# danieleschmidt/Photonic-Flash-Attention

Measured on AMD Instinct MI355X. Metric: attention_fwd_tflops, higher is better.
Workload: dtype bf16; 1 GPU; C3: B=4/GPU S=4096 H=16 D=128 bf16 causal (BASELINE.json configs[2], the headline shape); global_batch=4, seq_len=4096, heads=16, head_dim=128, causal=True, kernel=fa3_fwd_p4_bf16_d128_causal_o16, workgroups=256

## Files before the change

### include/pfa_hip.h

```cpp
#ifndef PFA_HIP_H
#define PFA_HIP_H

#include <stddef.h>
#include <stdint.h>

#ifdef __cplusplus
extern "C" {
#endif

#define PFA_ABI_VERSION 9

typedef enum pfa_status {
    PFA_OK = 0,
    PFA_ERR_NULL = -1,
    PFA_ERR_STRUCT_SIZE = -2,
    PFA_ERR_SHAPE = -3,
    PFA_ERR_HEAD_DIM = -4,
    PFA_ERR_DTYPE = -5,
    PFA_ERR_STRIDE = -6,
    PFA_ERR_ALIGN = -7,
    PFA_ERR_DEVICE = -8,
    PFA_ERR_LAUNCH = -9,
    PFA_ERR_FLAGS = -10
} pfa_status;

typedef enum pfa_dtype {
    PFA_DTYPE_BF16 = 0,
    PFA_DTYPE_FP16 = 1,
    PFA_DTYPE_FP32 = 2
} pfa_dtype;

#define PFA_FLAG_SPLIT_P   0x1u
#define PFA_FLAG_NO_XCD_MAP 0x2u
#define PFA_FLAG_VARIANT_MASK 0xff00u

typedef struct pfa_fa3_args {
    uint32_t size;
    uint32_t flags;

    const void* q;
    const void* k;
    const void* v;
    void*       o;
    float*      lse;
    const int32_t* seqlens_k;
    const uint8_t* key_mask;

    int64_t q_stride_b, q_stride_h, q_stride_s;
    int64_t k_stride_b, k_stride_h, k_stride_s;
    int64_t v_stride_b, v_stride_h, v_stride_s;
    int64_t o_stride_b, o_stride_h, o_stride_s;
    int64_t key_mask_stride_b;

    int32_t B, H, Sq, Sk, D;
    int32_t dtype_in;
    int32_t dtype_out;
// ... 304 lines not shown
```

### photonic_flash_attention_amd/_capi.py

```python

from __future__ import annotations

import ctypes as C
import os
import threading
from typing import Optional

PFA_ABI_VERSION = 9
PFA_DTYPE_BF16, PFA_DTYPE_FP16, PFA_DTYPE_FP32 = 0, 1, 2
PFA_FLAG_SPLIT_P = 0x1
PFA_FLAG_NO_XCD_MAP = 0x2
PFA_ROPE_INTERLEAVED = 0x1
PFA_MERGE_MAX_PARTS = 8
PFA_PREFILL_MAX_SPLITS = 8

_PKG_DIR = os.path.dirname(os.path.abspath(__file__))
LIB_PATH = os.path.join(_PKG_DIR, "libpfa_hip.so")

class PfaFa3Args(C.Structure):
    _fields_ = [
        ("size", C.c_uint32), ("flags", C.c_uint32),
        ("q", C.c_void_p), ("k", C.c_void_p), ("v", C.c_void_p), ("o", C.c_void_p),
        ("lse", C.c_void_p), ("seqlens_k", C.c_void_p), ("key_mask", C.c_void_p),
        ("q_stride_b", C.c_int64), ("q_stride_h", C.c_int64), ("q_stride_s", C.c_int64),
        ("k_stride_b", C.c_int64), ("k_stride_h", C.c_int64), ("k_stride_s", C.c_int64),
        ("v_stride_b", C.c_int64), ("v_stride_h", C.c_int64), ("v_stride_s", C.c_int64),
        ("o_stride_b", C.c_int64), ("o_stride_h", C.c_int64), ("o_stride_s", C.c_int64),
        ("key_mask_stride_b", C.c_int64),
        ("B", C.c_int32), ("H", C.c_int32), ("Sq", C.c_int32), ("Sk", C.c_int32), ("D", C.c_int32),
        ("dtype_in", C.c_int32), ("dtype_out", C.c_int32), ("causal", C.c_int32),
        ("softmax_scale", C.c_float), ("device_id", C.c_int32),
        ("workspace", C.c_void_p), ("workspace_bytes", C.c_size_t),
        ("mask", C.c_void_p),
        ("mask_stride_b", C.c_int64), ("mask_stride_h", C.c_int64), ("mask_stride_q", C.c_int64),
# ... 332 lines not shown
```

### photonic_flash_attention_amd/csrc/gen_fa3_fwd_p4.py

```python
#!/usr/bin/env python3
import os
import sys


DEV = os.environ.get("P4_DEV", "") == "1"
_stray = sorted(k for k in os.environ if k.startswith("P4_") and not (DEV and k in ("P4_DEV", "P4_STAMP")))
if _stray:
    sys.exit(f"gen_fa3_fwd_p4.py: {', '.join(_stray)} set without P4_DEV=1 -- the product code object takes no experiment knobs" if not DEV else
             f"gen_fa3_fwd_p4.py: unknown knob {', '.join(_stray)} -- P4_STAMP is the only one (with P4_DEV=1)")


def knob(name, default):
    return os.environ.get(name, default) if DEV else default


KA = dict(q=0, k=2, v=4, o=6, lse=8, q_sb=10, q_sh=11, k_sb=12, k_sh=13, v_sb=14, v_sh=15, o_sb=16, o_sh=17,
          q_ss=18, k_ss=19, v_ss=20, o_ss=21, H=22, Sq=23, Sk=24, NB=25, NU=26, magic_NU=27, magic_H=28, kv_group=29,
          magic_G=30, scale_log2=31, thr=32, hx=33, xcd_mode=34, SL=35, nt_full=36, pad=37, dbg=38)
KARG_DWORDS = 40
KARG_MEM_DWORDS = 42
KA_SEQLENS = 40
KBASE_SGPR = 60


# ... 115 lines not shown
    def need(self, tags):
        idx = [self.q.index(t) for t in tags if t in self.q]
        if not idx:
            return None
        i = max(idx)
        n = len(self.q) - 1 - i
        self.q = self.q[i + 1:]
        return f"s_waitcnt lgkmcnt({n})"


class Gen:
    def __init__(self, dtype, causal, out32=False, split=False, D=128, kmask=False, klen=False):
        assert out32 == split, "the code object carries the fast variant (16-bit store, one P) and the parity variant (fp32 store, split P)"
        self.dt, self.causal, self.out32, self.split, self.kmask = dtype, causal, out32, split, kmask
        self.klen = klen
        assert not (kmask and klen)
        self.kleft, self.kleft0 = (S('L_n'), ka('Sk')) if causal else (S('n_sub'), S('L_n'))
        self.mwords = kmask or klen
        self.nd_n, self.nd = S('nd_n'), S('nd')
        self.Lcut = S('L_n') if klen else ka('nt_full')
        if kmask and causal:
            self.kleft0 = ka('nt_full')
        self.cl = (klen or kmask) and causal
        self.fast = not split
        self.ret = S('grow')
        assert not (kmask and STAMP), "the key-mask kernels keep their mask words where the stamps keep their clock (s[58:59], the dbg kernarg)"
        assert D in (64, 128)
        self.D, self.KS, self.DB = D, D // 16, D // 32
        self.NKF, self.NVF = 2 * self.KS, 4 * self.DB
        self.TILE = 128 * D
        self.HALF = self.TILE // 2
        self.K_BASE, self.V_BASE, self.Q_BASE, self.O_BASE = 0, 2 * self.TILE, 4 * self.TILE, 8 * self.TILE
        self.LDS_BYTES = 10 * self.TILE
        self.PPW = self.TILE // 4096
        self.RB, self.CPR = 2 * D, D // 8
        assert RING <= min(self.NKF, self.NVF)
        self.mf = "v_mfma_f32_32x32x16_bf16" if dtype == "bf16" else "v_mfma_f32_32x32x16_f16"
        self.cvt = "v_cvt_pk_bf16_f32" if dtype == "bf16" else "v_cvt_pk_f16_f32"
        self.name = f"fa3_fwd_p4_{dtype}_d{D}_{'causal' if causal else 'full'}{'_km' if kmask else ('_kl' if klen else '')}_{'splitp_o32' if out32 else 'o16'}"
        self.main, self.ool, self.ool2, self.lstack = [], [], [], []
        self.L = self.main
        self.uid = 0

    def OA(self, X, db, e=0):
        return (0 if X == 'A' else 16 * self.DB) + 16 * db + e

# ... 460 lines not shown
                        self.i(x)
                        lg.issue(('kn', x))
                    pending = pending[2:]
                if rec is not None:
                    rec.append(sum(self.price(x.strip()) for x in self.L[mark:] if not x.strip().startswith("v_mfma")))
                else:
                    self.emit(fillers[hs] if hs < len(fillers) else [])
                hs += 1
        for x in pending:
            self.i(x)
        return lg

    def run_phase(self, fn, stream, lg, **kw):
        import copy
        save, uid = self.L, self.uid
        self.L, rec = [], []
        fn(fillers=None, lg=copy.deepcopy(lg), rec=rec, **kw)
        self.L, self.uid = save, uid
        fillers, tail = self.pack(stream, rec, ngaps=len(rec))
        lg = fn(fillers=fillers, lg=lg, **kw)
        self.emit(tail)
        return lg

    def stream_top(self, p):
        l1, l2 = self.ul("kok"), self.ul("vok")
        self.i(f"s_cmp_lg_u32 {S('krem')}, 0")
        self.i(f"s_cbranch_scc1 {l1}")
        self.i(f"s_mov_b64 {S('ksrd', 0, 2)}, {S('ksrd_n')}")
        self.i(f"s_mov_b32 {S('koff')}, 0")
        self.i(f"s_mov_b32 {S('krem')}, {S('nt_n')}")
        if self.kmask:
            self.i(f"s_mul_i32 {ka('pad')}, {S('n_b')}, {ka('Sk')}")
            self.i(f"s_mov_b32 {self.kleft}, {self.kleft0}")
        if self.klen:
            self.i(f"s_mov_b32 {ka('pad')}, {S('L_n')}")
        self.lab(l1)
        if self.kmask:
            self.len_word(0, dst=S('t2'), left=self.kleft)
            self.i(f"s_mov_b64 exec, {S('t2')}")
            self.emit(self.mask_load())
            self.i("s_mov_b64 exec, -1")
        if self.klen:
            self.len_word(p)
        self.i(f"s_cmp_lg_u32 {S('vrem')}, 0")
        self.i(f"s_cbranch_scc1 {l2}")
        self.i(f"s_mov_b64 {S('vsrd', 0, 2)}, {S('vsrd_n')}")
        self.i(f"s_mov_b32 {S('voff')}, 0")
        self.i(f"s_mov_b32 {S('vrem')}, {S('nt_n')}")
        self.lab(l2)

    def capture(self, fn):
        save, self.L = self.L, []
        fn()
        out, self.L = self.L, save
        return [x[1:] if x.startswith("\t") else x for x in out]

    def stream_bottom(self, p, barrier=True):
        lq, lb = self.ul("q"), self.ul("bar")
        self.i(f"s_add_u32 {S('koff')}, {S('koff')}, {S('ktile')}")
        self.i(f"s_add_u32 {S('voff')}, {S('voff')}, {S('vtile')}")
        self.i(f"s_sub_u32 {S('krem')}, {S('krem')}, 1")
        self.i(f"s_sub_u32 {S('vrem')}, {S('vrem')}, 1")
        self.i(f"s_sub_u32 {S('wrem')}, {S('wrem')}, 1")
        if self.kmask:
            self.i(f"s_add_u32 {ka('pad')}, {ka('pad')}, 64")
        if self.klen:
            self.i(f"s_sub_u32 {ka('pad')}, {ka('pad')}, 64")
        self.i(f"s_cmp_lg_u32 {S('qrem')}, 0")
        self.i(f"s_cbranch_scc1 {lq}")
        self.i("s_waitcnt vmcnt(0)")
        self.lab(lb)
        if self.kmask:
            self.i(self.mask_word(p))
            self.km_len_and(p)
        if barrier:
            self.i("s_barrier")
        self.out_of_line(True)
        self.lab(lq)
        self.q_group()
        self.q_group()
        self.i("s_waitcnt vmcnt(8)")
        self.i(f"s_branch {lb}")
        self.out_of_line(False)
# ... 81 lines not shown
            self.i(f"s_cmp_eq_u32 {S('wrem')}, {self.nd if self.cl else 1}")
            self.i(f"s_cbranch_scc1 {lm}")
            self.lab(lr)
            self.out_of_line(True)
            self.lab(lm)
            self.mask_diag(1 - p)
            self.i(f"s_branch {lr}")
            self.out_of_line(False)
        if not self.fast:
            sta = self.interleave(self.start_stream('A', 1 - p), self.start_stream('B', 1 - p, alt=True))
            self.run_phase(self.phase_pv, sta, lg, p=p, dma_at={}, preissued=True)
            lr, lb = self.ul("rescale"), self.ul("rescaled")
            self.i(f"s_cmp_lg_u64 {S('grow')}, 0")
            self.i(f"s_cbranch_scc1 {lr}")
            self.lab(lb)
            self.out_of_line(True)
            self.lab(lr)
            self.rescale()
            self.i(f"s_branch {lb}")
            self.out_of_line(False)
            return
        sta = self.interleave(self.start_fast('A', 1 - p), self.start_fast('B', 1 - p))
        if lean:
            inline = [f"s_add_u32 {S('koff')}, {S('koff')}, {S('ktile')}", f"s_add_u32 {S('voff')}, {S('voff')}, {S('vtile')}"] + \
                     ([f"s_add_u32 {ka('pad')}, {ka('pad')}, 64"] if self.kmask else []) + ["s_waitcnt vmcnt(0)"] + \
                     ([self.mask_word(p)] if self.kmask else [])
        else:
            inline = self.capture(lambda: self.stream_bottom(p, barrier=False))
        mid = dict(gap=MID_BARRIER_GAP[self.D], inline=inline, kreads=self.kprefetch(p))
        self.run_phase(self.phase_pv, sta, lg, p=p, dma_at={}, preissued=True, mid=mid)

    def body_last(self, p):
        self.cm(f"LAST body, parity {p}: this wave's last tile -- finish(j), PV(j); nothing to prefetch for the wave itself")
        d = self.dma_plan(p, [2 * t for t in range(self.PPW)], [2 * self.PPW + 2 * t for t in range(self.PPW)])
        if self.fast:
            self.emit(self.finish_fast(p))
            self.fix_check(p)
            self.emit(self.lupd('A') + self.lupd('B'))
            self.i("s_nop 1")
            self.phase_pv(p, [[] for _ in range(2 * self.NVF)], d, strips="AB")
            return
        self.emit(self.finish_stream('A', p))
        self.i("s_nop 1")
        self.run_phase(self.phase_pv, self.finish_stream('B', p), Lgkm(), p=p, dma_at=d, strips="A")
        self.i("s_nop 1")
        self.phase_pv(p, [[] for _ in range(2 * self.NVF)], {}, strips="B")

# ... 566 lines not shown
            self.i(f"v_lshlrev_b32 {e2}, 4, {e2}")
            for d, ss in ((KDOFF(t), 'k_ss'), (VDOFF(t), 'v_ss')):
                self.i(f"v_mul_lo_u32 {e4}, {e3}, {ka(ss)}")
                self.i(f"v_add_u32 {e4}, {e4}, {e2}")
                self.i(f"v_subrev_u32 {vr(d)}, {1024 * t}, {e4}")
        self.i(f"s_lshl_b32 {S('t1')}, {W}, 6")
        for t in range(4):
            self.i(f"v_lshl_or_b32 {e2}, {e0}, 2, {t}")
            self.i(f"v_xor_b32 {e2}, {e2}, {e1}")
            self.i(f"v_add_u32 {e3}, {4 * t}, {e0}")
            self.i(f"v_lshrrev_b32 {e4}, 3, {e2}")
            self.i(f"v_lshl_add_u32 {e3}, {e3}, 1, {e4}")
            self.i(f"v_add_u32 {e3}, {S('t1')}, {e3}")
            self.i(f"v_and_b32 {e2}, 7, {e2}")
            self.i(f"v_lshlrev_b32 {e2}, 4, {e2}")
            self.i(f"v_mul_lo_u32 {e4}, {e3}, {ka('q_ss')}")
            self.i(f"v_add_u32 {e4}, {e4}, {e2}")
            self.i(f"v_subrev_u32 {vr(QDOFF(t))}, {1024 * t}, {e4}")

    def item_switch(self):
        self.i(f"s_mov_b32 {S('irem')}, {S('n_nt')}")
        self.i(f"s_sub_u32 {S('krem')}, {S('n_nt')}, 2")
        self.i(f"s_sub_u32 {S('vrem')}, {S('n_nt')}, 1")
        if self.cl:
            self.i(f"s_cmp_eq_u32 {self.nd_n}, 0")
            self.i(f"s_cselect_b32 {S('wrem')}, {S('wave')}, 3")
            self.i(f"s_cselect_b32 {self.nd}, 1, 0x80000000")
            self.i(f"s_add_u32 {S('wrem')}, {S('wrem')}, {S('n_nt')}")
            self.i(f"s_sub_u32 {S('wrem')}, {S('wrem')}, 4")
        elif self.causal:
            self.i(f"s_add_u32 {S('wrem')}, {S('n_nt')}, {S('wave')}")
            self.i(f"s_sub_u32 {S('wrem')}, {S('wrem')}, 4")
        else:
            self.i(f"s_sub_u32 {S('wrem')}, {S('n_nt')}, 1")
        self.make_out_srds()
        if self.causal:
            lone, ldone = self.ul("loneblock"), self.ul("advanced")
            self.i(f"s_lshl_b32 {S('t0')}, {S('n_qblk')}, 1")
            self.i(f"s_add_u32 {S('t0')}, {S('t0')}, 1")
            self.i(f"s_sub_u32 {S('t0')}, {S('t0')}, {ka('NB')}")
            self.i(f"s_or_b32 {S('t0')}, {S('t0')}, {S('n_sub')}")
            self.i(f"s_cmp_eq_u32 {S('t0')}, 0")
            self.i(f"s_cbranch_scc1 {lone}")
            self.i(f"s_xor_b32 {S('n_sub')}, {S('n_sub')}, 1")
            self.i(f"s_cmp_eq_u32 {S('n_sub')}, 0")
            self.i(f"s_cselect_b32 {S('t0')}, 1, 0")
            self.i(f"s_add_u32 {S('n_u')}, {S('n_u')}, {S('t0')}")
            self.i(f"s_branch {ldone}")
            self.lab(lone)
            self.i(f"s_add_u32 {S('n_u')}, {S('n_u')}, 1")
            self.lab(ldone)
        else:
            self.i(f"s_add_u32 {S('n_u')}, {S('n_u')}, 1")
        self.decode()
        self.i(f"s_mov_b32 {S('nt_n')}, {S('n_nt')}")
        self.i(f"s_lshl_b32 {S('qrem')}, {S('n_valid')}, {2 if self.PPW == 4 else 1}")
        self.i(f"s_lshl_b32 {S('qdst')}, {S('w4k')}, 2")
        self.i(f"s_add_u32 {S('qdst')}, {S('qdst')}, {self.Q_BASE}")
        self.i(f"s_mov_b32 {S('qoff')}, 0")

    def kernel(self):
        n = self.name
        self.L += [f"\t.globl\t{n}", "\t.p2align\t8", f"\t.type\t{n},@function", f"{n}:"]
        self.i(f"s_load_dwordx16 s[{KBASE_SGPR}:{KBASE_SGPR + 15}], s[0:1], 0")
        self.i(f"s_load_dwordx16 s[{KBASE_SGPR + 16}:{KBASE_SGPR + 31}], s[0:1], 64")
        self.i(f"s_load_dwordx8 s[{KBASE_SGPR + 32}:{KBASE_SGPR + 39}], s[0:1], 128")
        L, T0, T1, T2, T3 = vr(V_LANE), *(vr(x) for x in V_T)
        W = S('wave')
        self.i(f"v_and_b32 {L}, 63, v0")
        self.i(f"v_lshrrev_b32 {T0}, 6, v0")
        self.i("s_nop 0")
        self.i(f"v_readfirstlane_b32 {W}, {T0}")
        self.i("s_waitcnt lgkmcnt(0)")
        self.stamp_init()
        self.i(f"s_lshl_b32 {S('ktile')}, {ka('k_ss')}, 6")
        self.i(f"s_lshl_b32 {S('vtile')}, {ka('v_ss')}, 6")
        self.i(f"s_lshl_b32 {S('w4k')}, {W}, {12 if self.D == 128 else 11}")
        for sr, ss, rows in (('ksrd', 'k_ss', 'Sk'), ('vsrd', 'v_ss', 'Sk'), ('qsrd_n', 'q_ss', None), ('osrd', 'o_ss', None)):
# ... 26 lines not shown
        self.i(f"s_cbranch_scc1 {lend}")
        self.i(f"s_lshl_b32 {S('qdst')}, {S('w4k')}, 2")
        self.i(f"s_add_u32 {S('qdst')}, {S('qdst')}, {self.Q_BASE}")
        self.i(f"s_mov_b32 {S('qoff')}, 0")
        if self.kmask:
            self.i(f"s_mul_i32 {ka('pad')}, {S('n_b')}, {ka('Sk')}")
            self.emit(self.mask_load(0))
            self.i(f"s_add_u32 {ka('pad')}, {ka('pad')}, 64")
            self.emit(self.mask_load(1))
            self.i(f"s_add_u32 {ka('pad')}, {ka('pad')}, 64")
        if self.klen:
            self.i(f"s_mov_b32 {ka('pad')}, {S('L_n')}")
            self.len_word(0)
            self.i(f"s_sub_u32 {ka('pad')}, {ka('pad')}, 64")
            self.len_word(1)
            self.i(f"s_sub_u32 {ka('pad')}, {ka('pad')}, 64")
        self.i(f"s_mov_b32 {S('qrem')}, {self.PPW}")
        for g in range(self.PPW):
            self.q_group()
        self.i(f"s_mov_b64 {S('ksrd', 0, 2)}, {S('ksrd_n')}")
        self.i(f"s_mov_b64 {S('vsrd', 0, 2)}, {S('vsrd_n')}")
        self.i(f"s_mov_b32 {S('koff')}, 0")
        self.i(f"s_mov_b32 {S('voff')}, 0")
        self.i(self.setm0('k', 0))
        self.i("s_nop 0")
        for t in range(self.PPW):
            self.i(self.dma('K', t))
        self.i(self.setm0('v', 0))
        self.i("s_nop 0")
        for t in range(self.PPW):
            self.i(self.dma('V', t))
        self.i(f"s_add_u32 {S('koff')}, {S('koff')}, {S('ktile')}")
        self.i(self.setm0('k', 1))
        self.i("s_nop 0")
        for t in range(self.PPW):
            self.i(self.dma('K', t))
        self.i(f"s_add_u32 {S('koff')}, {S('koff')}, {S('ktile')}")
        self.i(f"s_add_u32 {S('voff')}, {S('voff')}, {S('vtile')}")
        self.i(f"s_waitcnt vmcnt({2 * self.PPW})")
        if self.kmask:
            self.i(self.mask_word(0, 0))
            self.i(self.mask_word(1, 1))
            self.i(f"s_mov_b32 {self.kleft}, {self.kleft0}")
            self.km_len_and(0)
            self.km_len_and(1)
        self.i("s_barrier")
        litem = f".L{n}_item"
        self.lab(litem)
        self.item_switch()
        self.item_prologue()
        self.i("s_waitcnt vmcnt(0)")
        self.i("s_barrier")
        if self.fast:
            self.emit(self.kprefetch(1))
        lloop, lgen, lseam = f".L{n}_loop", f".L{n}_generic", f".L{n}_seam"
        self.lab(lloop)
        self.i(f"s_cmp_lt_u32 {S('krem')}, {(5 if self.causal else 2) + (2 if self.mwords else 0)}")
        self.i(f"s_cbranch_scc1 {lgen}")
        self.i(f"s_cmp_lg_u32 {S('qrem')}, 0")
        self.i(f"s_cbranch_scc1 {lgen}")
        for p in (0, 1):
            if self.kmask:
                self.emit(self.mask_load())
            self.body_full(p, lean=True)
            if self.fast:
                continue
            self.i(f"s_add_u32 {S('koff')}, {S('koff')}, {S('ktile')}")
            self.i(f"s_add_u32 {S('voff')}, {S('voff')}, {S('vtile')}")
            if self.kmask:
                self.i(f"s_add_u32 {ka('pad')}, {ka('pad')}, 64")
            self.i("s_waitcnt vmcnt(0)")
            if self.kmask:
                self.i(self.mask_word(p))
            self.i("s_barrier")
        for c in ("krem", "vrem", "wrem", "irem"):
            self.i(f"s_sub_u32 {S(c)}, {S(c)}, 2")
        if self.kmask:
            self.i(f"s_sub_u32 {self.kleft}, {self.kleft}, 128")
        if self.klen:
            self.i(f"s_mov_b64 {self.MK(0)}, -1")
            self.i(f"s_mov_b64 {self.MK(1)}, -1")
            self.i(f"s_sub_u32 {ka('pad')}, {ka('pad')}, 128")
        self.i(f"s_branch {lloop}")
        self.lab(lgen)
        for p in (0, 1):
            lnf, ll, ld = (self.ul(x) for x in ("notfull", "last", "done"))
            if p == 1:
                lnorm = self.ul("noseam")
                self.i(f"s_cmp_eq_u32 {S('irem')}, 2")
                self.i(f"s_cbranch_scc0 {lnorm}")
                self.i(f"s_cmp_lg_u32 {S('n_valid')}, 0")
# ... 143 lines not shown
```

### photonic_flash_attention_amd/csrc/pfa_capi.hip

```cpp
#include "pfa_hip.h"

#include <hip/hip_runtime.h>
#include <math.h>
#include <stdio.h>
#include <string.h>

#include "fa3_fwd_kernel.h"
#include "fa3_weights_kernel.h"
#include "fa3_fwd_f32_kernel.h"
#include "pfa_host.h"
#include "pfa_mask_host.h"
#include "pfa_p4.h"

namespace pfa { const void* w4_kernel(int dtype, bool causal, bool out32); }

namespace {

thread_local int g_last_hip_error = 0;

struct Variant {
    const void* fn;
    char name[96];
    int lds_bytes;
    bool grid3 = false;
// ... 48 lines not shown
    const int hpx = (a->B * a->H) % 8 == 0 ? (a->B * a->H) / 8 : 0;
    v.xcd_group = (hpx > 0 && hpx % 4 == 0) ? 4 : ((hpx > 0 && hpx % 2 == 0) ? 2 : 0);
    return v;
}

Variant pick(const pfa_fa3_args* a) {
    const bool causal = a->causal != 0, split = (a->flags & PFA_FLAG_SPLIT_P) != 0;
    const bool kmask = a->key_mask != nullptr || a->mask != nullptr;
    const bool out32 = a->dtype_out == PFA_DTYPE_FP32;
    const unsigned var = (a->flags >> 8) & 0xffu;
    const bool w4_ok = a->D == 128 && !split && !kmask && (int64_t)a->B * a->H * a->H < (1ll << 32);
    const int64_t avg_tiles = (causal ? (int64_t)a->Sk / 2 : (int64_t)a->Sk) / pfa::BLOCK_N;
    if (pfa::p4_eligible(a) && (var == 45 || var == 0)) {
        Variant v = p4_variant(a, causal);
        if (v.p4_grid > 0) return v;
    }
    if (w4_ok && (var == 43 || ((var == 0 || var == 45) && avg_tiles >= 16))) return w4_variant(a, causal, out32);
    return w8_variant(a, causal, split, kmask, out32);
}

int check(const pfa_fa3_args* a) {
    if (!a) return PFA_ERR_NULL;
    if (a->size != sizeof(pfa_fa3_args)) return PFA_ERR_STRUCT_SIZE;
    if (a->flags & ~(PFA_FLAG_SPLIT_P | PFA_FLAG_NO_XCD_MAP | PFA_FLAG_VARIANT_MASK)) return PFA_ERR_FLAGS;
    {
        const unsigned var = (a->flags & PFA_FLAG_VARIANT_MASK) >> 8;
        if (var != 0 && var != 43 && var != 44 && var != 45) return PFA_ERR_FLAGS;
    }
    if (!a->q || !a->k || !a->v || !a->o) return PFA_ERR_NULL;
    if (a->key_mask && a->mask) return PFA_ERR_FLAGS;
    if (a->kv_group < 0 || a->reserve_cus < 0 || a->reserved1 != 0 || (a->kv_group > 1 && a->H % a->kv_group != 0)) return PFA_ERR_SHAPE;
    if (a->drop_mask && (a->dtype_in != PFA_DTYPE_FP32 || !(a->drop_scale >= 1.f) || !isfinite(a->drop_scale))) return PFA_ERR_FLAGS;
    if (a->B <= 0 || a->H <= 0 || a->Sq <= 0 || a->Sk <= 0) return PFA_ERR_SHAPE;
    if (a->D != 64 && a->D != 128) return PFA_ERR_HEAD_DIM;
    if (a->dtype_in != PFA_DTYPE_BF16 && a->dtype_in != PFA_DTYPE_FP16 && a->dtype_in != PFA_DTYPE_FP32) return PFA_ERR_DTYPE;
    if (a->dtype_out != a->dtype_in && a->dtype_out != PFA_DTYPE_FP32) return PFA_ERR_DTYPE;
    using pfa::aligned16; using pfa::aligned4; using pfa::slab_fits32;
    const int32_t Sq = a->Sq, Sk = a->Sk, D = a->D;
    if (a->dtype_in == PFA_DTYPE_FP32) {
        if (a->flags & (PFA_FLAG_SPLIT_P | PFA_FLAG_VARIANT_MASK)) return PFA_ERR_FLAGS;
        if (!pfa::qkv_strides_multiples_of(4, a)) return PFA_ERR_STRIDE;
        if (!aligned16(a->q) || !aligned16(a->k) || !aligned16(a->v) || !aligned4(a->o)) return PFA_ERR_ALIGN;
        if (!pfa::scale_ok(a->softmax_scale)) return PFA_ERR_SHAPE;
        if ((int64_t)((Sq + 63) / 64) * a->B * a->H > 0x7fffffffLL) return PFA_ERR_SHAPE;
        if (!aligned4(a->lse)) return PFA_ERR_ALIGN;
        if (a->q_stride_s < D || a->k_stride_s < D || a->v_stride_s < D || a->o_stride_s < D) return PFA_ERR_STRIDE;
        if (!slab_fits32(Sq, a->q_stride_s, D, 4) || !slab_fits32(Sk, a->k_stride_s, D, 4) || !slab_fits32(Sk, a->v_stride_s, D, 4) ||
            !slab_fits32(Sq, a->o_stride_s, D, 4))
            return PFA_ERR_SHAPE;
        return PFA_OK;
    }
    if (!pfa::scale_ok(a->softmax_scale)) return PFA_ERR_SHAPE;
    if (!pfa::qkv_strides_multiples_of(8, a) || !pfa::multiples_of(4, {a->o_stride_b, a->o_stride_h, a->o_stride_s})) return PFA_ERR_STRIDE;
    if (!aligned16(a->q) || !aligned16(a->k) || !aligned16(a->v) || !aligned16(a->o) || !aligned4(a->lse)) return PFA_ERR_ALIGN;
    if ((int64_t)((Sq + 127) / 128) * a->B * a->H > 0x7fffffffLL) return PFA_ERR_SHAPE;
    if (!slab_fits32(Sk, a->k_stride_s, D, 2) || !slab_fits32(Sk, a->v_stride_s, D, 2) || !slab_fits32(Sq, a->q_stride_s, D, 2)) return PFA_ERR_SHAPE;
    if (!pfa::kv_rows_forward(a) || a->k_stride_s * 64 > 0x3fffffffLL || a->v_stride_s * 64 > 0x3fffffffLL) return PFA_ERR_STRIDE;
    return PFA_OK;
}

pfa::MaskWords mask_words(const pfa_fa3_args* a) {
    return a->key_mask ? pfa::mask_words(a->key_mask, a->B, 1, 1, a->Sk, a->key_mask_stride_b, 0, 0, 1) : pfa::element_mask_words(a);
}
// ... 179 lines not shown
```

### photonic_flash_attention_amd/csrc/pfa_p4.hip

```cpp
#include <hip/hip_runtime.h>
#include <stddef.h>
#include <stdint.h>
#include <stdio.h>
#include <string.h>

#include <mutex>

#include "pfa_hip.h"
#include "pfa_host.h"
#include "pfa_p4.h"
#include "build/fa3_fwd_p4_offsets.h"

__asm__(".section .rodata\n"
        ".global pfa_p4_hsaco_begin\n.global pfa_p4_hsaco_end\n"
        ".balign 4096\n"
        "pfa_p4_hsaco_begin:\n"
        ".incbin \"" PFA_P4_HSACO_PATH "\"\n"
        "pfa_p4_hsaco_end:\n"
        ".byte 0\n"
        ".previous\n");
extern "C" const unsigned char pfa_p4_hsaco_begin[];
extern "C" const unsigned char pfa_p4_hsaco_end[];

namespace pfa {

struct P4Params {
    const void* q;
    const void* k;
    const void* v;
    void* o;
    float* lse;
    uint32_t q_sb, q_sh, k_sb, k_sh, v_sb, v_sh, o_sb, o_sh;
    uint32_t q_ss, k_ss, v_ss, o_ss;
    uint32_t H, Sq, Sk, NB, NU, magic_NU, magic_H, kv_group, magic_G;
    float scale_log2, thr;
    uint32_t hx, xcd_mode, SL, nt_full, pad;
    unsigned long long* dbg;
    const int32_t* seqlens_k;
};
#define P4_CHECK(field, macro) static_assert(offsetof(P4Params, field) == macro, "kernarg layout of " #field)
P4_CHECK(q, P4_KA_Q); P4_CHECK(k, P4_KA_K); P4_CHECK(v, P4_KA_V); P4_CHECK(o, P4_KA_O); P4_CHECK(lse, P4_KA_LSE);
P4_CHECK(q_sb, P4_KA_Q_SB); P4_CHECK(q_sh, P4_KA_Q_SH); P4_CHECK(k_sb, P4_KA_K_SB); P4_CHECK(k_sh, P4_KA_K_SH);
P4_CHECK(v_sb, P4_KA_V_SB); P4_CHECK(v_sh, P4_KA_V_SH); P4_CHECK(o_sb, P4_KA_O_SB); P4_CHECK(o_sh, P4_KA_O_SH);
P4_CHECK(q_ss, P4_KA_Q_SS); P4_CHECK(k_ss, P4_KA_K_SS); P4_CHECK(v_ss, P4_KA_V_SS); P4_CHECK(o_ss, P4_KA_O_SS);
P4_CHECK(H, P4_KA_H); P4_CHECK(Sq, P4_KA_SQ); P4_CHECK(Sk, P4_KA_SK); P4_CHECK(NB, P4_KA_NB); P4_CHECK(NU, P4_KA_NU);
P4_CHECK(magic_NU, P4_KA_MAGIC_NU); P4_CHECK(magic_H, P4_KA_MAGIC_H); P4_CHECK(kv_group, P4_KA_KV_GROUP);
P4_CHECK(magic_G, P4_KA_MAGIC_G); P4_CHECK(scale_log2, P4_KA_SCALE_LOG2); P4_CHECK(thr, P4_KA_THR); P4_CHECK(hx, P4_KA_HX);
P4_CHECK(xcd_mode, P4_KA_XCD_MODE); P4_CHECK(SL, P4_KA_SL); P4_CHECK(nt_full, P4_KA_NT_FULL); P4_CHECK(dbg, P4_KA_DBG);
P4_CHECK(seqlens_k, P4_KA_SEQLENS);
static_assert(sizeof(P4Params) == P4_KARG_BYTES, "kernarg size");

namespace {
constexpr int MAX_DEV = 64;
struct DevMod {
    hipModule_t mod = nullptr;
    hipFunction_t fn[2][2][2][3][2] = {};
    int n_cu = 0;
    int state = 0;
    int last_err = 0;
};
DevMod g_mod[MAX_DEV];
std::mutex g_mu;

uint32_t magic(uint32_t d) { return d <= 1 ? 0u : (uint32_t)((1ull << 32) / d) + 1u; }

const DevMod* module_for(int dev, int* hip_err = nullptr) {
    if (dev < 0 || dev >= MAX_DEV) return nullptr;
    DevMod& m = g_mod[dev];
    if (__atomic_load_n(&m.state, __ATOMIC_ACQUIRE) == 1) return &m;
    std::lock_guard<std::mutex> lk(g_mu);
    if (m.state == 0) {
// ... 91 lines not shown
    P4Params p;
    memset(&p, 0, sizeof(p));
    p.q = a->q; p.k = a->k; p.v = a->v; p.o = a->o; p.lse = a->lse;
    p.q_sb = (uint32_t)(a->q_stride_b * 2); p.q_sh = (uint32_t)(a->q_stride_h * 2); p.q_ss = (uint32_t)(a->q_stride_s * 2);
    p.k_sb = (uint32_t)(a->k_stride_b * 2); p.k_sh = (uint32_t)(a->k_stride_h * 2); p.k_ss = (uint32_t)(a->k_stride_s * 2);
    p.v_sb = (uint32_t)(a->v_stride_b * 2); p.v_sh = (uint32_t)(a->v_stride_h * 2); p.v_ss = (uint32_t)(a->v_stride_s * 2);
    const bool parity = a->dtype_out == PFA_DTYPE_FP32;
    const int64_t osz = parity ? 4 : 2;
    p.o_sb = (uint32_t)(a->o_stride_b * osz); p.o_sh = (uint32_t)(a->o_stride_h * osz); p.o_ss = (uint32_t)(a->o_stride_s * osz);
    p.H = (uint32_t)a->H; p.Sq = (uint32_t)a->Sq; p.Sk = (uint32_t)a->Sk;
    p.NB = (uint32_t)((a->Sq + 255) / 256);
    p.NU = a->causal ? (p.NB + 1) / 2 : p.NB;
    p.magic_NU = magic(p.NU); p.magic_H = magic(p.H);
    p.kv_group = (uint32_t)kv_group_of(a);
    p.magic_G = magic(p.kv_group);
    p.scale_log2 = a->softmax_scale * pfa::LOG2E;
    p.thr = 8.0f / p.scale_log2;
    const int BH = a->B * a->H;
    const int grid = grid_for(m, a);
    p.xcd_mode = BH % 8 == 0 ? 1u : 0u;
    p.hx = p.xcd_mode ? (uint32_t)(BH / 8) : (uint32_t)BH;
    p.SL = p.xcd_mode ? (uint32_t)(grid / 8) : (uint32_t)grid;
    p.nt_full = (uint32_t)(((a->Sk + 127) / 128) * 2);
    p.dbg = (a->workspace && a->workspace_bytes >= (size_t)grid * 4 * 16 * 4) ? (unsigned long long*)a->workspace : nullptr;
    if (a->key_mask) p.dbg = (unsigned long long*)a->key_mask;
    p.seqlens_k = a->seqlens_k;

    size_t sz = sizeof(p);
    void* config[] = {HIP_LAUNCH_PARAM_BUFFER_POINTER, &p, HIP_LAUNCH_PARAM_BUFFER_SIZE, &sz, HIP_LAUNCH_PARAM_END};
    hipFunction_t fn = m->fn[a->dtype_in == PFA_DTYPE_BF16 ? 0 : 1][a->D == 64 ? 1 : 0][a->causal ? 1 : 0][p4_flavour(a)][parity ? 1 : 0];
    const DeviceScope dev(a->device_id);
    if (hip_failed(dev.error(), hip_err)) return PFA_ERR_DEVICE;
    const hipError_t e = hipModuleLaunchKernel(fn, (unsigned)grid, 1, 1, 256, 1, 1, 0, (hipStream_t)stream, nullptr, config);
    return hip_failed(e, hip_err) ? PFA_ERR_LAUNCH : PFA_OK;
}

}
```

### photonic_flash_attention_amd/ops.py

```python

from __future__ import annotations

import ctypes as C
import operator
import threading
from typing import Optional, Tuple

import torch

from . import _capi

_DT = {torch.bfloat16: _capi.PFA_DTYPE_BF16, torch.float16: _capi.PFA_DTYPE_FP16, torch.float32: _capi.PFA_DTYPE_FP32}

SUPPORTED_HEAD_DIMS = (64, 128)


def _padded_head_dim(D: int) -> int:
    if D in SUPPORTED_HEAD_DIMS:
        return D
    if 1 <= D < SUPPORTED_HEAD_DIMS[-1]:
        return next(d for d in SUPPORTED_HEAD_DIMS if d > D)
    raise ValueError(f"head_dim {D} has no kernel (<= {SUPPORTED_HEAD_DIMS[-1]} supported)")


# ... 100 lines not shown

def _scale(softmax_scale: Optional[float], D: int) -> float:
    return float(D ** -0.5 if softmax_scale is None else softmax_scale)


_ARANGE1 = {}


def _mask_bound(km: torch.Tensor) -> torch.Tensor:
    if km.is_cuda and torch.cuda.is_current_stream_capturing():
        idx = torch.arange(1, km.shape[1] + 1, dtype=torch.int32, device=km.device)
        return (idx * (km != 0)).amax(dim=1).to(torch.int32)
    key = (km.shape[1], str(km.device))
    with _SEQLENS_LOCK:
        idx = _ARANGE1.get(key)
        if idx is None:
            if len(_ARANGE1) > 64:
                _ARANGE1.clear()
            idx = _ARANGE1[key] = torch.arange(1, km.shape[1] + 1, dtype=torch.int32, device=km.device)
    return (idx * (km != 0)).amax(dim=1).to(torch.int32)


def build_args(q, k, v, out, *, causal=False, seqlens_k=None, key_mask=None, softmax_scale=None,
               lse=None, split_p=False, variant=0, mask=None, drop_mask=None, drop_scale=1.0):
    B, H, Sq, D = q.shape
    Sk, Hkv = k.shape[2], k.shape[1]
    if Hkv < 1 or H % Hkv or k.shape != (B, Hkv, Sk, D) or v.shape != (B, Hkv, Sk, D):
        raise ValueError(f"shape mismatch: q {tuple(q.shape)} k {tuple(k.shape)} v {tuple(v.shape)}")
    if out.shape != (B, H, Sq, D):
        raise ValueError("output shape mismatch")
    if q.dtype not in (torch.bfloat16, torch.float16, torch.float32) or k.dtype != q.dtype or v.dtype != q.dtype:
        raise ValueError("q, k, v must share dtype bf16, fp16 or fp32 (fp32: the exact, slow kernel)")
    if out.dtype not in (q.dtype, torch.float32):
        raise ValueError("output dtype must be the input dtype or fp32")
    if q.dtype == torch.float32 and (split_p or variant):
        raise ValueError("fp32 operands run the exact fp32 kernel: no split P, no kernel selector")
    if not (q.is_cuda and k.is_cuda and v.is_cuda and out.is_cuda):
        raise ValueError("pfa_fa3_fwd needs device tensors (there is no CPU path)")
    a = _capi.make_args(
        flags=(_capi.PFA_FLAG_SPLIT_P if split_p else 0) | ((int(variant) & 0xFF) << 8),
        B=B, H=H, Sq=Sq, Sk=Sk, D=D,
        dtype_in=_DT[q.dtype], dtype_out=_DT[out.dtype], causal=1 if causal else 0,
        softmax_scale=_scale(softmax_scale, D),
        device_id=_device_index(q.device),
        kv_group=H // Hkv,
    )
    _set_strides(a, (("q", q), ("k", k), ("v", v), ("o", out)))
    keep = []
    if seqlens_k is not None:
        sl = _seqlens_tensor(seqlens_k, q.device)
        if sl.numel() != B:
            raise ValueError("seqlens_k must have B entries")
        a.seqlens_k = sl.data_ptr()
        keep.append(sl)
    if key_mask is not None:
        km = key_mask
        if km.shape != (B, Sk):
            raise ValueError("key_mask must be [B, Sk]")
        if km.dtype == torch.bool and km.device == q.device:
            km = km.contiguous().view(torch.uint8)
        else:
            km = (km != 0).to(device=q.device, dtype=torch.uint8).contiguous()
        a.key_mask = km.data_ptr()
# ... 7 lines not shown
    if mask is not None:
        if key_mask is not None:
            raise ValueError("pass either key_mask or mask")
        _set_element_mask(a, mask, B, H, Sq, Sk, q.device, keep)
    if key_mask is not None or mask is not None:
        ws_bytes = int(_capi.load().pfa_fa3_workspace_bytes(C.byref(a)))
        if ws_bytes:
            ws = torch.empty(ws_bytes, dtype=torch.uint8, device=q.device)
            a.workspace, a.workspace_bytes = ws.data_ptr(), ws_bytes
            keep.append(ws)
    if lse is not None:
        a.lse = _lse_ptr(lse, B, H, Sq)
    if drop_mask is not None:
        a.drop_mask, a.drop_scale = _drop_mask_ptr(drop_mask, B, H, Sq, Sk, q), float(drop_scale)
        keep.append(drop_mask)
    return a, keep


def fa3_forward(q: torch.Tensor, k: torch.Tensor, v: torch.Tensor, *, causal: bool = False,
                seqlens_k=None, key_mask: Optional[torch.Tensor] = None, mask: Optional[torch.Tensor] = None,
                softmax_scale: Optional[float] = None, out_dtype: Optional[torch.dtype] = None,
                return_lse: bool = False, return_weights: bool = False, weights_dtype: Optional[torch.dtype] = None,
                split_p: Optional[bool] = None, drop_mask: Optional[torch.Tensor] = None, drop_scale: float = 1.0,
                out: Optional[torch.Tensor] = None, _variant: Optional[int] = None) -> Tuple[torch.Tensor, Optional[torch.Tensor]]:
    B, H, Sq, D = q.shape
    Dp = _padded_head_dim(D)
    if Dp != D:
        res = fa3_forward(_pad_d(q, Dp), _pad_d(k, Dp), _pad_d(v, Dp), causal=causal, seqlens_k=seqlens_k,
                          key_mask=key_mask, mask=mask,
                          softmax_scale=_scale(softmax_scale, D), out_dtype=out_dtype,
                          return_lse=return_lse, return_weights=return_weights, weights_dtype=weights_dtype,
                          split_p=split_p, drop_mask=drop_mask, drop_scale=drop_scale, _variant=_variant)
        o = res[0][..., :D]
        if out is not None:
            out.copy_(o)
            o = out
        return (o,) + tuple(res[1:])
    if _variant is None:
        _variant = 0
    odt = q.dtype if out_dtype is None else out_dtype
    if q.dtype == torch.float32:
        if return_weights:
            raise ValueError("return_weights with fp32 operands: call again with 16-bit operands for the weights")
        if split_p or _variant:
            raise ValueError("fp32 operands run the exact fp32 kernel: no split P, no kernel selector")
        split_p = False
    elif split_p is None:
        split_p = odt == torch.float32
    if out is None:
        out = torch.empty((B, Sq, H, D), dtype=odt, device=q.device).permute(0, 2, 1, 3)
    lse = torch.empty((B, H, Sq), dtype=torch.float32, device=q.device) if (return_lse or return_weights) else None
    args, keep = build_args(q, k, v, out, causal=causal, seqlens_k=seqlens_k, key_mask=key_mask, mask=mask,
                            softmax_scale=softmax_scale, lse=lse, split_p=split_p, variant=_variant,
                            drop_mask=drop_mask, drop_scale=drop_scale)
    stream = torch.cuda.current_stream(q.device).cuda_stream
    st = _capi.load().pfa_fa3_fwd(C.byref(args), C.c_void_p(stream))
    _raise_status("pfa_fa3_fwd", st)
    weights = None
    if return_weights:
        Sk = k.shape[2]
        wdt = q.dtype if weights_dtype is None else weights_dtype
        weights = torch.empty((B, H, Sq, Sk), dtype=wdt, device=q.device)
        stw = _capi.load().pfa_fa3_weights(C.byref(args), C.c_void_p(weights.data_ptr()), _DT[wdt],
                                           weights.stride(0), weights.stride(1), weights.stride(2), C.c_void_p(stream))
        _raise_status("pfa_fa3_weights", stw)
    for t in keep:
        t.record_stream(torch.cuda.current_stream(q.device))
    if return_weights:
        return out, (lse if return_lse else None), weights
    return out, lse


def fa3_forward_bshd(q, k, v, **kw):
    res = fa3_forward(q.permute(0, 2, 1, 3), k.permute(0, 2, 1, 3), v.permute(0, 2, 1, 3), **kw)
    return (res[0].permute(0, 2, 1, 3),) + tuple(res[1:])

# ... 904 lines not shown
```

Measured before the change: 1245 TFLOP/s.

## Stream causal K/V tiles in descending order for light work units

```diff
diff --git a/include/pfa_hip.h b/include/pfa_hip.h
--- a/include/pfa_hip.h
+++ b/include/pfa_hip.h
@@ -32,6 +32,7 @@
 
 #define PFA_FLAG_SPLIT_P   0x1u
 #define PFA_FLAG_NO_XCD_MAP 0x2u
+#define PFA_FLAG_LIGHT_ASCENDING 0x4u
 #define PFA_FLAG_VARIANT_MASK 0xff00u
 
 typedef struct pfa_fa3_args {
diff --git a/photonic_flash_attention_amd/_capi.py b/photonic_flash_attention_amd/_capi.py
--- a/photonic_flash_attention_amd/_capi.py
+++ b/photonic_flash_attention_amd/_capi.py
@@ -10,6 +10,7 @@
 PFA_DTYPE_BF16, PFA_DTYPE_FP16, PFA_DTYPE_FP32 = 0, 1, 2
 PFA_FLAG_SPLIT_P = 0x1
 PFA_FLAG_NO_XCD_MAP = 0x2
+PFA_FLAG_LIGHT_ASCENDING = 0x4
 PFA_ROPE_INTERLEAVED = 0x1
 PFA_MERGE_MAX_PARTS = 8
 PFA_PREFILL_MAX_SPLITS = 8
diff --git a/photonic_flash_attention_amd/csrc/gen_fa3_fwd_p4.py b/photonic_flash_attention_amd/csrc/gen_fa3_fwd_p4.py
--- a/photonic_flash_attention_amd/csrc/gen_fa3_fwd_p4.py
+++ b/photonic_flash_attention_amd/csrc/gen_fa3_fwd_p4.py
@@ -161,6 +161,11 @@
         if kmask and causal:
             self.kleft0 = ka('nt_full')
         self.cl = (klen or kmask) and causal
+        self.desc = causal and not kmask and not klen
+        if self.desc:
+            self.kstep, self.vstep, self.dsc_n, self.jt = S('nd_n'), S('nd'), S('L_n'), ka('nt_full')
+        else:
+            self.kstep, self.vstep = S('ktile'), S('vtile')
         self.fast = not split
         self.ret = S('grow')
         assert not (kmask and STAMP), "the key-mask kernels keep their mask words where the stamps keep their clock (s[58:59], the dbg kernarg)"
@@ -667,12 +672,44 @@
         self.emit(tail)
         return lg
 
+    def stream_start(self, off, step, tile):
+        if not self.desc:
+            self.i(f"s_mov_b32 {off}, 0")
+            return
+        self.i(f"s_mul_i32 {off}, {self.dsc_n}, {tile}")
+        self.i(f"s_sub_u32 {step}, 0, {tile}")
+        self.i(f"s_cmp_eq_u32 {self.dsc_n}, 0")
+        self.i(f"s_cselect_b32 {step}, {tile}, {step}")
+
+    def stream_turn(self, off, step, tile, rem, lj, ld):
+        self.out_of_line(True)
+        self.lab(lj)
+        self.i(f"s_cmp_eq_u32 {rem}, 4")
+        self.i(f"s_cbranch_scc0 {ld}")
+        self.i(f"s_cmp_lt_i32 {step}, 0")
+        self.i(f"s_cbranch_scc0 {ld}")
+        self.i(f"s_mul_i32 {off}, {self.jt}, {tile}")
+        self.i(f"s_mov_b32 {step}, {tile}")
+        self.i(f"s_branch {ld}")
+        self.out_of_line(False)
+
+    def stream_event(self, rem, ld):
+        if not self.desc:
+            self.i(f"s_cmp_lg_u32 {rem}, 0")
+            self.i(f"s_cbranch_scc1 {ld}")
+            return None
+        lj = self.ul("turn")
+        self.i(f"s_cmp_gt_u32 {rem}, 4")
+        self.i(f"s_cbranch_scc1 {ld}")
+        self.i(f"s_cmp_lg_u32 {rem}, 0")
+        self.i(f"s_cbranch_scc1 {lj}")
+        return lj
+
     def stream_top(self, p):
         l1, l2 = self.ul("kok"), self.ul("vok")
-        self.i(f"s_cmp_lg_u32 {S('krem')}, 0")
-        self.i(f"s_cbranch_scc1 {l1}")
+        lj = self.stream_event(S('krem'), l1)
         self.i(f"s_mov_b64 {S('ksrd', 0, 2)}, {S('ksrd_n')}")
-        self.i(f"s_mov_b32 {S('koff')}, 0")
+        self.stream_start(S('koff'), self.kstep, S('ktile'))
         self.i(f"s_mov_b32 {S('krem')}, {S('nt_n')}")
         if self.kmask:
             self.i(f"s_mul_i32 {ka('pad')}, {S('n_b')}, {ka('Sk')}")
@@ -680,6 +717,8 @@
         if self.klen:
             self.i(f"s_mov_b32 {ka('pad')}, {S('L_n')}")
         self.lab(l1)
+        if lj:
+            self.stream_turn(S('koff'), self.kstep, S('ktile'), S('krem'), lj, l1)
         if self.kmask:
             self.len_word(0, dst=S('t2'), left=self.kleft)
             self.i(f"s_mov_b64 exec, {S('t2')}")
@@ -687,12 +726,13 @@
             self.i("s_mov_b64 exec, -1")
         if self.klen:
             self.len_word(p)
-        self.i(f"s_cmp_lg_u32 {S('vrem')}, 0")
-        self.i(f"s_cbranch_scc1 {l2}")
+        lj = self.stream_event(S('vrem'), l2)
         self.i(f"s_mov_b64 {S('vsrd', 0, 2)}, {S('vsrd_n')}")
-        self.i(f"s_mov_b32 {S('voff')}, 0")
+        self.stream_start(S('voff'), self.vstep, S('vtile'))
         self.i(f"s_mov_b32 {S('vrem')}, {S('nt_n')}")
         self.lab(l2)
+        if lj:
+            self.stream_turn(S('voff'), self.vstep, S('vtile'), S('vrem'), lj, l2)
 
     def capture(self, fn):
         save, self.L = self.L, []
@@ -702,8 +742,8 @@
 
     def stream_bottom(self, p, barrier=True):
         lq, lb = self.ul("q"), self.ul("bar")
-        self.i(f"s_add_u32 {S('koff')}, {S('koff')}, {S('ktile')}")
-        self.i(f"s_add_u32 {S('voff')}, {S('voff')}, {S('vtile')}")
+        self.i(f"s_add_u32 {S('koff')}, {S('koff')}, {self.kstep}")
+        self.i(f"s_add_u32 {S('voff')}, {S('voff')}, {self.vstep}")
         self.i(f"s_sub_u32 {S('krem')}, {S('krem')}, 1")
         self.i(f"s_sub_u32 {S('vrem')}, {S('vrem')}, 1")
         self.i(f"s_sub_u32 {S('wrem')}, {S('wrem')}, 1")
@@ -831,7 +871,7 @@
             return
         sta = self.interleave(self.start_fast('A', 1 - p), self.start_fast('B', 1 - p))
         if lean:
-            inline = [f"s_add_u32 {S('koff')}, {S('koff')}, {S('ktile')}", f"s_add_u32 {S('voff')}, {S('voff')}, {S('vtile')}"] + \
+            inline = [f"s_add_u32 {S('koff')}, {S('koff')}, {self.kstep}", f"s_add_u32 {S('voff')}, {S('voff')}, {self.vstep}"] + \
                      ([f"s_add_u32 {ka('pad')}, {ka('pad')}, 64"] if self.kmask else []) + ["s_waitcnt vmcnt(0)"] + \
                      ([self.mask_word(p)] if self.kmask else [])
         else:
@@ -1444,6 +1484,8 @@
         self.i(f"s_mov_b32 {S('irem')}, {S('n_nt')}")
         self.i(f"s_sub_u32 {S('krem')}, {S('n_nt')}, 2")
         self.i(f"s_sub_u32 {S('vrem')}, {S('n_nt')}, 1")
+        if self.desc:
+            self.i(f"s_sub_u32 {self.jt}, {S('n_nt')}, 4")
         if self.cl:
             self.i(f"s_cmp_eq_u32 {self.nd_n}, 0")
             self.i(f"s_cselect_b32 {S('wrem')}, {S('wave')}, 3")
@@ -1476,6 +1518,13 @@
             self.i(f"s_add_u32 {S('n_u')}, {S('n_u')}, 1")
         self.decode()
         self.i(f"s_mov_b32 {S('nt_n')}, {S('n_nt')}")
+        if self.desc:
+            self.i(f"s_sub_u32 {self.dsc_n}, {S('n_nt')}, 5")
+            self.i(f"s_and_b32 {S('t0')}, {S('n_valid')}, {ka('pad')}")
+            self.i(f"s_mul_i32 {S('t0')}, {S('t0')}, {S('n_sub')}")
+            self.i(f"s_mul_i32 {self.dsc_n}, {self.dsc_n}, {S('t0')}")
+            self.i(f"s_cmp_eq_u32 {S('n_qblk')}, 0")
+            self.i(f"s_cselect_b32 {self.dsc_n}, 0, {self.dsc_n}")
         self.i(f"s_lshl_b32 {S('qrem')}, {S('n_valid')}, {2 if self.PPW == 4 else 1}")
         self.i(f"s_lshl_b32 {S('qdst')}, {S('w4k')}, 2")
         self.i(f"s_add_u32 {S('qdst')}, {S('qdst')}, {self.Q_BASE}")
@@ -1548,6 +1597,12 @@
         self.i(f"s_mov_b64 {S('vsrd', 0, 2)}, {S('vsrd_n')}")
         self.i(f"s_mov_b32 {S('koff')}, 0")
         self.i(f"s_mov_b32 {S('voff')}, 0")
+        if self.desc:
+            for _ in range(6):
+                self.i("s_nop 0")
+            self.i(f"s_mov_b32 {self.kstep}, {S('ktile')}")
+            self.i(f"s_mov_b32 {self.vstep}, {S('vtile')}")
+            self.i(f"s_mov_b32 {self.dsc_n}, 0")
         self.i(self.setm0('k', 0))
         self.i("s_nop 0")
         for t in range(self.PPW):
@@ -1581,7 +1636,7 @@
             self.emit(self.kprefetch(1))
         lloop, lgen, lseam = f".L{n}_loop", f".L{n}_generic", f".L{n}_seam"
         self.lab(lloop)
-        self.i(f"s_cmp_lt_u32 {S('krem')}, {(5 if self.causal else 2) + (2 if self.mwords else 0)}")
+        self.i(f"s_cmp_lt_u32 {S('krem')}, {(6 if self.desc else 5 if self.causal else 2) + (2 if self.mwords else 0)}")
         self.i(f"s_cbranch_scc1 {lgen}")
         self.i(f"s_cmp_lg_u32 {S('qrem')}, 0")
         self.i(f"s_cbranch_scc1 {lgen}")
@@ -1591,8 +1646,8 @@
             self.body_full(p, lean=True)
             if self.fast:
                 continue
-            self.i(f"s_add_u32 {S('koff')}, {S('koff')}, {S('ktile')}")
-            self.i(f"s_add_u32 {S('voff')}, {S('voff')}, {S('vtile')}")
+            self.i(f"s_add_u32 {S('koff')}, {S('koff')}, {self.kstep}")
+            self.i(f"s_add_u32 {S('voff')}, {S('voff')}, {self.vstep}")
             if self.kmask:
                 self.i(f"s_add_u32 {ka('pad')}, {ka('pad')}, 64")
             self.i("s_waitcnt vmcnt(0)")
diff --git a/photonic_flash_attention_amd/csrc/pfa_capi.hip b/photonic_flash_attention_amd/csrc/pfa_capi.hip
--- a/photonic_flash_attention_amd/csrc/pfa_capi.hip
+++ b/photonic_flash_attention_amd/csrc/pfa_capi.hip
@@ -94,7 +94,7 @@
 int check(const pfa_fa3_args* a) {
     if (!a) return PFA_ERR_NULL;
     if (a->size != sizeof(pfa_fa3_args)) return PFA_ERR_STRUCT_SIZE;
-    if (a->flags & ~(PFA_FLAG_SPLIT_P | PFA_FLAG_NO_XCD_MAP | PFA_FLAG_VARIANT_MASK)) return PFA_ERR_FLAGS;
+    if (a->flags & ~(PFA_FLAG_SPLIT_P | PFA_FLAG_NO_XCD_MAP | PFA_FLAG_LIGHT_ASCENDING | PFA_FLAG_VARIANT_MASK)) return PFA_ERR_FLAGS;
     {
         const unsigned var = (a->flags & PFA_FLAG_VARIANT_MASK) >> 8;
         if (var != 0 && var != 43 && var != 44 && var != 45) return PFA_ERR_FLAGS;
@@ -110,7 +110,7 @@
     using pfa::aligned16; using pfa::aligned4; using pfa::slab_fits32;
     const int32_t Sq = a->Sq, Sk = a->Sk, D = a->D;
     if (a->dtype_in == PFA_DTYPE_FP32) {
-        if (a->flags & (PFA_FLAG_SPLIT_P | PFA_FLAG_VARIANT_MASK)) return PFA_ERR_FLAGS;
+        if (a->flags & (PFA_FLAG_SPLIT_P | PFA_FLAG_LIGHT_ASCENDING | PFA_FLAG_VARIANT_MASK)) return PFA_ERR_FLAGS;
         if (!pfa::qkv_strides_multiples_of(4, a)) return PFA_ERR_STRIDE;
         if (!aligned16(a->q) || !aligned16(a->k) || !aligned16(a->v) || !aligned4(a->o)) return PFA_ERR_ALIGN;
         if (!pfa::scale_ok(a->softmax_scale)) return PFA_ERR_SHAPE;
diff --git a/photonic_flash_attention_amd/csrc/pfa_p4.hip b/photonic_flash_attention_amd/csrc/pfa_p4.hip
--- a/photonic_flash_attention_amd/csrc/pfa_p4.hip
+++ b/photonic_flash_attention_amd/csrc/pfa_p4.hip
@@ -34,7 +34,8 @@
     uint32_t q_ss, k_ss, v_ss, o_ss;
     uint32_t H, Sq, Sk, NB, NU, magic_NU, magic_H, kv_group, magic_G;
     float scale_log2, thr;
-    uint32_t hx, xcd_mode, SL, nt_full, pad;
+    uint32_t hx, xcd_mode, SL, nt_full;
+    uint32_t pad;
     unsigned long long* dbg;
     const int32_t* seqlens_k;
 };
@@ -46,7 +47,8 @@
 P4_CHECK(H, P4_KA_H); P4_CHECK(Sq, P4_KA_SQ); P4_CHECK(Sk, P4_KA_SK); P4_CHECK(NB, P4_KA_NB); P4_CHECK(NU, P4_KA_NU);
 P4_CHECK(magic_NU, P4_KA_MAGIC_NU); P4_CHECK(magic_H, P4_KA_MAGIC_H); P4_CHECK(kv_group, P4_KA_KV_GROUP);
 P4_CHECK(magic_G, P4_KA_MAGIC_G); P4_CHECK(scale_log2, P4_KA_SCALE_LOG2); P4_CHECK(thr, P4_KA_THR); P4_CHECK(hx, P4_KA_HX);
-P4_CHECK(xcd_mode, P4_KA_XCD_MODE); P4_CHECK(SL, P4_KA_SL); P4_CHECK(nt_full, P4_KA_NT_FULL); P4_CHECK(dbg, P4_KA_DBG);
+P4_CHECK(xcd_mode, P4_KA_XCD_MODE); P4_CHECK(SL, P4_KA_SL); P4_CHECK(nt_full, P4_KA_NT_FULL); P4_CHECK(pad, P4_KA_PAD);
+P4_CHECK(dbg, P4_KA_DBG);
 P4_CHECK(seqlens_k, P4_KA_SEQLENS);
 static_assert(sizeof(P4Params) == P4_KARG_BYTES, "kernarg size");
 
@@ -184,6 +186,7 @@
     p.hx = p.xcd_mode ? (uint32_t)(BH / 8) : (uint32_t)BH;
     p.SL = p.xcd_mode ? (uint32_t)(grid / 8) : (uint32_t)grid;
     p.nt_full = (uint32_t)(((a->Sk + 127) / 128) * 2);
+    p.pad = (a->flags & PFA_FLAG_LIGHT_ASCENDING) ? 0u : 1u;
     p.dbg = (a->workspace && a->workspace_bytes >= (size_t)grid * 4 * 16 * 4) ? (unsigned long long*)a->workspace : nullptr;
     if (a->key_mask) p.dbg = (unsigned long long*)a->key_mask;
     p.seqlens_k = a->seqlens_k;
diff --git a/photonic_flash_attention_amd/ops.py b/photonic_flash_attention_amd/ops.py
--- a/photonic_flash_attention_amd/ops.py
+++ b/photonic_flash_attention_amd/ops.py
@@ -146,7 +146,7 @@
 
 
 def build_args(q, k, v, out, *, causal=False, seqlens_k=None, key_mask=None, softmax_scale=None,
-               lse=None, split_p=False, variant=0, mask=None, drop_mask=None, drop_scale=1.0):
+               lse=None, split_p=False, variant=0, mask=None, drop_mask=None, drop_scale=1.0, light_ascending=False):
     B, H, Sq, D = q.shape
     Sk, Hkv = k.shape[2], k.shape[1]
     if Hkv < 1 or H % Hkv or k.shape != (B, Hkv, Sk, D) or v.shape != (B, Hkv, Sk, D):
@@ -162,7 +162,7 @@
     if not (q.is_cuda and k.is_cuda and v.is_cuda and out.is_cuda):
         raise ValueError("pfa_fa3_fwd needs device tensors (there is no CPU path)")
     a = _capi.make_args(
-        flags=(_capi.PFA_FLAG_SPLIT_P if split_p else 0) | ((int(variant) & 0xFF) << 8),
+        flags=(_capi.PFA_FLAG_SPLIT_P if split_p else 0) | ((int(variant) & 0xFF) << 8) | (_capi.PFA_FLAG_LIGHT_ASCENDING if light_ascending else 0),
         B=B, H=H, Sq=Sq, Sk=Sk, D=D,
         dtype_in=_DT[q.dtype], dtype_out=_DT[out.dtype], causal=1 if causal else 0,
         softmax_scale=_scale(softmax_scale, D),
@@ -216,7 +216,8 @@
                 softmax_scale: Optional[float] = None, out_dtype: Optional[torch.dtype] = None,
                 return_lse: bool = False, return_weights: bool = False, weights_dtype: Optional[torch.dtype] = None,
                 split_p: Optional[bool] = None, drop_mask: Optional[torch.Tensor] = None, drop_scale: float = 1.0,
-                out: Optional[torch.Tensor] = None, _variant: Optional[int] = None) -> Tuple[torch.Tensor, Optional[torch.Tensor]]:
+                out: Optional[torch.Tensor] = None, _variant: Optional[int] = None,
+                _light_ascending: bool = False) -> Tuple[torch.Tensor, Optional[torch.Tensor]]:
     B, H, Sq, D = q.shape
     Dp = _padded_head_dim(D)
     if Dp != D:
@@ -245,7 +246,7 @@
         out = torch.empty((B, Sq, H, D), dtype=odt, device=q.device).permute(0, 2, 1, 3)
     lse = torch.empty((B, H, Sq), dtype=torch.float32, device=q.device) if (return_lse or return_weights) else None
     args, keep = build_args(q, k, v, out, causal=causal, seqlens_k=seqlens_k, key_mask=key_mask, mask=mask,
-                            softmax_scale=softmax_scale, lse=lse, split_p=split_p, variant=_variant,
+                            softmax_scale=softmax_scale, lse=lse, split_p=split_p, variant=_variant, light_ascending=_light_ascending,
                             drop_mask=drop_mask, drop_scale=drop_scale)
     stream = torch.cuda.current_stream(q.device).cuda_stream
     st = _capi.load().pfa_fa3_fwd(C.byref(args), C.c_void_p(stream))
```

After: 1245 TFLOP/s, median of 2. About the same (-0.0%).
